# psipred/DMPfold2

Hardware: AMD Instinct MI355X
Metric: structures/s at L=300, N_seq=2000, 10 iters+100 min (higher is better)
Workload: dtype f32 with full-width operands on the bf16 matrix cores (option precision = 2): convolution operands split exactly into 3 bf16 pieces (24 significand bits), the 6 piece products above 2^-24 accumulated in f32 by v_mfma_f32_32x32x16_bf16; vertical GRU the same way (3 bf16 pieces per operand, 6 products

## Files before the change

dmpfold2_amd/csrc/api.hip:

```cpp
#include "cluster.h"
#include <atomic>
#include "conv_bf16.h"
#include "conv_f16.h"
#include <cstdarg>
#include <cstdio>
#include <cstring>
#include <cmath>

namespace dmp {

static thread_local char g_err[512] = "";

void set_error(const char* fmt, ...) {
  va_list ap;
  va_start(ap, fmt);
  vsnprintf(g_err, sizeof(g_err), fmt, ap);
  va_end(ap);
}

int hip_fail(hipError_t e, const char* what, const char* file, int line) {
  set_error("HIP error %d (%s) at %s:%d: %s", (int)e, hipGetErrorString(e), file, line, what);
  return DMP_ERR_HIP;
}

// ... 251 lines not shown
    }
    for (int q = 0; q < 128; ++q) {
      float a = 0.f;
      for (int r = 0; r < 8; ++r) a += w2[q * 8 + r] * hid[r];
      gate[q] = 1.0f / (1.0f + std::exp(-a));
    }
    if ((rc = upload(pool, bytes, &B.cse, gate))) return rc;
    {
      std::vector<float> fc(w1);
      fc.insert(fc.end(), w2.begin(), w2.end());
      if ((rc = upload(pool, bytes, &B.cse_fc, fc))) return rc;
    }
    if ((rc = upload(pool, bytes, &B.sse_w, H[p + ".scSE.sSE.conv.weight"]))) return rc;
    B.sse_b = H[p + ".scSE.sSE.conv.bias"][0];
  }
  if ((rc = upload(pool, bytes, &W.head_w, H["resnet.17.weight"]))) return rc;
  W.head_b[0] = H["resnet.17.bias"][0];
  W.head_b[1] = H["resnet.17.bias"][1];
  return DMP_OK;
}

static int check_ready(dmp_ctx* c, int L, int N) {
  if (!c) { set_error("null context"); return DMP_ERR_ARG; }
  if (L > c->max_L || N > c->max_N) {
    set_error("alignment %d x %d exceeds the context capacity %d x %d", N, L, c->max_N, c->max_L);
    return DMP_ERR_CAPACITY;
  }
  return DMP_OK;
}
static int need_weights(dmp_ctx* c) {
  if (!c->W.ready) { set_error("weights not finalized"); return DMP_ERR_WEIGHTS; }
  return DMP_OK;
}

static int trunk_open(dmp_ctx* c, const float* z0, const float* dmap, int L, hipStream_t s) {
  int rc;
  c->trunk_cur = c->xa;
  c->trunk_oth = c->xb;
  c->xsplit_current = false;
  c->ab_current = false;
  if ((rc = stem_update_padded(c, z0, dmap, L, c->trunk_cur, s, true))) return rc;
  c->xsplit_current = c->conv_mode != 1;
  return DMP_OK;
}

static int trunk_block(dmp_ctx* c, int k, int L, hipStream_t s) {
  int rc;
  {
    static const int depth = getenv("DMP_LANE_DEPTH") ? std::max(1, atoi(getenv("DMP_LANE_DEPTH"))) : 2;
    if (c->lane && c->lane->count >= depth)
      DMP_HIP(hipStreamWaitEvent(s, (hipEvent_t)c->lane->ev[(c->lane->count - depth) % dmp_lane::RING], 0));
  }
  if (c->prof_on && c->prof_n + 2 <= (int)c->prof_ev.size()) {
    DMP_HIP(hipEventRecord((hipEvent_t)c->prof_ev[c->prof_n], s));
  }
  if ((rc = conv5x5_maxout_padded(c, k, c->trunk_cur, L, c->u, c->stats, s, false))) return rc;
  if (c->lane) {
    dmp_lane* ln = c->lane;
    void* e = ln->ev[ln->next];
    ln->next = (ln->next + 1) % dmp_lane::RING;
    DMP_HIP(hipEventRecord((hipEvent_t)e, s));
    ln->last = e;
    ln->count++;
  }
  if (c->prof_on && c->prof_n + 2 <= (int)c->prof_ev.size()) {
    DMP_HIP(hipEventRecord((hipEvent_t)c->prof_ev[c->prof_n + 1], s));
    c->prof_n += 2;
  }
  if ((rc = conv5x5_reduce_stats(c, L, c->stats, s, k))) return rc;
  if ((rc = norm_scse_residual_padded(c, k, c->u, c->stats, c->trunk_cur, L, c->trunk_oth, s, k == NBLOCK))) return rc;
  std::swap(c->trunk_cur, c->trunk_oth);
  return DMP_OK;
}

static int trunk_close(dmp_ctx* c, int L, float* d_conf, float* d_M, hipStream_t s) {
  c->xsplit_current = false;
  return head_gram_padded(c, c->trunk_cur, L, d_conf, d_M, s);
}

static int trunk_pass(dmp_ctx* c, const float* z0, const float* dmap, int L, float* d_conf,
                      float* d_M, hipStream_t s) {
  struct Reset { dmp_ctx* c; ~Reset() { c->xsplit_current = false; } } reset{c};
  int rc;
  if ((rc = trunk_open(c, z0, dmap, L, s))) return rc;
  for (int k = 1; k <= NBLOCK; ++k)
    if ((rc = trunk_block(c, k, L, s))) return rc;
  return trunk_close(c, L, d_conf, d_M, s);
}

static int coords_from_mds(dmp_ctx* c, const float* mat1d, const float* mds, int L, float* d_ca,
                           hipStream_t s) {
  int rc;
  if ((rc = build_embed(mat1d, mds, L, c->emb, s))) return rc;
  if ((rc = gru_bidir(c, 1, c->emb, L, c->seq_a, s))) return rc;
  return coord_fc(c, c->seq_a, L, d_ca, s);
}

__global__ void fault_latch_kernel(int* __restrict__ words, float* __restrict__ coords,
                                   float* __restrict__ conf, int L, ConfLayout lay, int* __restrict__ report) {
  const int f = words[0];
  if (!f) return;
  const int64_t i = (int64_t)blockIdx.x * blockDim.x + threadIdx.x;
  const float nan = __builtin_nanf("");
  if (i < 15 * L) coords[i] = nan;
  if (conf_is_out(lay, i)) conf[i] = nan;
  if (i == 0) {
    atomicOr(&words[1], f);
    if (report) *report = f;
  }
}

static int scratch_reserve(dmp_ctx* c, Scratch& w, int64_t need, int64_t head, const char* what) {
  if (w.p && w.bytes >= need) return DMP_OK;
  int prev = 0;
  DMP_HIP(hipGetDevice(&prev));
  DMP_HIP(hipSetDevice(c->device));
  void* p = nullptr;
  hipError_t e = hipMalloc(&p, (size_t)need);
  if (e == hipSuccess) e = hipMemset(p, 0, (size_t)head);
  if (e == hipSuccess && w.p) e = hipFree(w.p);
  (void)hipSetDevice(prev);
  if (e != hipSuccess) {
    if (p) (void)hipFree(p);
    return hip_fail(e, what, __FILE__, __LINE__);
  }
  c->bytes += need - w.bytes;
  w = {(unsigned char*)p, need};
  return DMP_OK;
}
static int scratch_reserve(dmp_ctx* c, Scratch& w, ScratchNeed n, const char* what) { return scratch_reserve(c, w, n.bytes, n.head, what); }

static int search_reserve(dmp_ctx* c) {
  if (c->opt.search <= 0) return DMP_OK;
  const int mm = c->opt.search_mm > 0 ? c->opt.search_mm : c->max_L;
  int64_t need = 0;
  for (int L = 8; L <= c->max_L; ++L)
    need = std::max<int64_t>(need, (int64_t)search_chunk_entries(L, mm, 0) * search_slot(L, mm).total);
  return scratch_reserve(c, c->search_ws, SEARCH_HEAD_BYTES + need, SEARCH_HEAD_BYTES, "search scratch");
}
static int search_domains_reserve(dmp_ctx* c) {
  return c->opt.search_domains ? scratch_reserve(c, c->domsearch_ws, search_domains_need(c->max_L), "domain-search scratch") : DMP_OK;
}
static int passes_reserve(dmp_ctx* c) {
  return c->opt.passes ? scratch_reserve(c, c->pass_ws, score_passes_need(c->max_L), "pass-score scratch") : DMP_OK;
}
static int with_entity_reserve(dmp_ctx* c, Scratch& w, ScratchNeed n, const char* what) {
  const bool had = c->entity_ws.p != nullptr;
  int rc = scratch_reserve(c, c->entity_ws, entity_need(c->max_L), "native-entity scratch");
  if (!rc && (rc = scratch_reserve(c, w, n, what)) && !had) {
    (void)hipFree(c->entity_ws.p);
    c->bytes -= c->entity_ws.bytes;
    c->entity_ws = {};
  }
  return rc;
}
static int ss_reserve(dmp_ctx* c) {
  return c->opt.ss ? with_entity_reserve(c, c->ss_ws, assign_ss_need(c->max_L), "secondary-structure scratch") : DMP_OK;
}
static int exposure_reserve(dmp_ctx* c) {
  return c->opt.exposure ? with_entity_reserve(c, c->exposure_ws, exposure_need(c->max_L), "exposure scratch") : DMP_OK;
}
static int domains_reserve(dmp_ctx* c) {
  return c->opt.domains ? with_entity_reserve(c, c->domains_ws, domains_need(c->max_L), "domain scratch") : DMP_OK;
}

enum OptAccess { OPT_RW, OPT_READ_ONLY , OPT_GET_ONLY  };
// ... 973 lines not shown

int dmp_predict_end(dmp_ctx* ctx, float* d_coords, float* d_conf, void* stream) {
  DMP_ARG(ctx && d_coords && d_conf, "null argument");
  dmp_ctx* c = ctx;
  int rc = predict_end_refine(ctx, stream);
  if (rc) return rc;
  hipStream_t s = STREAM;
  const int L = c->last_L;
  rc = ca_to_backbone(c->best_ca, c->best_conf, L, d_coords, d_conf, s);
  if (rc) return rc;
  const int pass_R = c->run.passes ? std::min(c->run_depth + 1, c->max_passes) : 0;
  const ConfLayout lay = conf_layout(L, c->run, pass_R);
  if (c->run.emit && (rc = emit_distmap(c, c->best_ca, L, c->passes_done, d_conf + lay.map.off, d_conf + lay.info.off, s))) return rc;
  if (c->run.score && (rc = score_native(c, d_coords, L, d_conf + lay.score.off, s))) return rc;
  if (c->run.smap && (rc = score_map(c, L, d_conf + lay.score.off, d_conf + lay.smap.off, s))) return rc;
  if (pass_R && (rc = score_passes(c, L, pass_R, std::min(c->passes_done, c->max_passes), d_conf + lay.pass.off, s))) return rc;
  const float* d_native = c->run.score ? d_conf + lay.score.off : nullptr;
  const bool backbone = c->run.ss || c->run.exposure;
  if (d_native && (backbone || c->run.domains) && (rc = entity_prepare(c, d_native, L, backbone, s))) return rc;
  if (c->run.ss && (rc = assign_ss(c, d_coords, L, d_native, d_conf + lay.ss.off, s))) return rc;
  if (c->run.exposure && (rc = exposure(c, d_coords, L, d_native, d_conf + lay.exposure.off, s))) return rc;
  if (c->run.domains && (rc = domains(c, d_coords, L, d_native, d_conf + lay.domains.off, s))) return rc;
  if (c->run.align && (rc = align_structure(c, d_coords, L, d_conf + lay.align.off, s))) return rc;
  if (c->run.search > 0 && (rc = search_structures(c, d_coords, L, d_conf, lay, s))) return rc;
  if (c->run.search_domains && (rc = search_domains(c, d_coords, L, d_conf, lay, s))) return rc;
  hipLaunchKernelGGL(fault_latch_kernel, dim3((unsigned)cdiv64(std::max<int64_t>(15 * L, lay.total), 256)), dim3(256), 0, s,
                     c->seq_abort, d_coords, d_conf, L, lay, c->end_fault_out);
  DMP_LAUNCH_CHECK();
  return DMP_OK;
}

static std::shared_ptr<dmp_lane> lane_create() {
  std::shared_ptr<dmp_lane> l(new dmp_lane(), [](dmp_lane* p) {
    for (void* e : p->ev) (void)hipEventDestroy((hipEvent_t)e);
    delete p;
  });
  for (int i = 0; i < dmp_lane::RING; ++i) {
    hipEvent_t e;
    if (hipEventCreateWithFlags(&e, hipEventDisableTiming) != hipSuccess) return nullptr;
    l->ev.push_back((void*)e);
  }
  return l;
}

int dmp_ctx_share_lane(dmp_ctx* ctx, dmp_ctx* other) {
  DMP_ARG(ctx != nullptr, "null context");
  if (!other) { ctx->lane_hold.reset(); ctx->lane = nullptr; return DMP_OK; }
  DMP_ARG(other != ctx && other->device == ctx->device, "a lane is shared by different contexts of one GPU");
  if (!other->lane_hold) {
    other->lane_hold = lane_create();
    if (!other->lane_hold) { set_error("hipEventCreate failed for the lane"); return DMP_ERR_HIP; }
    other->lane = other->lane_hold.get();
  }
  ctx->lane_hold = other->lane_hold;
  ctx->lane = ctx->lane_hold.get();
  return DMP_OK;
}

int64_t dmp_debug_fetch(dmp_ctx* ctx, const char* name, float* d_dst, int64_t capacity, void* stream) {
  DMP_ARG(ctx && name && d_dst, "null argument");
  const int64_t L = ctx->last_L, N = ctx->last_N;
  const int64_t P = std::min(ctx->passes_done, ctx->max_passes);
  const float* src = nullptr;
  int64_t n = 0;
  const std::string k(name);
  if (k == "w") { src = ctx->w; n = N; }
  else if (k == "contacts") { src = ctx->contacts; n = L * L; }
  else if (k == "mat1d") { src = ctx->mat1d; n = WIDTH * L; }
  else if (k == "conf_means") { src = ctx->conf_means; n = P; }
  else if (k == "ca_pass") { src = ctx->ca_pass; n = P * L * 3; }
  else if (k == "pass_delta") { src = ctx->pass_delta; n = ctx->run.tol_mA > 0 ? P : 0; }
  else if (k == "best_dm") { src = ctx->best_dm; n = ctx->run.emit || ctx->run.restrain > 0 ? L * L : 0; }
  else if (k == "best_pass") { src = ctx->best_pass; n = 1; }
  else if (k == "best_ca") { src = ctx->best_ca_snapshot; n = L * 3; }
  else if (k == "best_ca_refined") { src = ctx->best_ca; n = L * 3; }
  else if (k == "inv_cov") { src = ctx->cov; n = (int64_t)NS * L * NS * L; }
  else if (k == "mds") { src = ctx->mds; n = L * 8; }
  else if (k == "gram") { src = ctx->gram; n = L * L; }
  else if (k == "vgru_h0" || k == "vgru_h1") {
    const int layer = k == "vgru_h1";
    src = ctx->hT[layer][ctx->vg_maxN & 1];
    n = (int64_t)WIDTH * ctx->vg_ntiles * 32;
  }
  else if (k == "exposure_points") return exposure_points_fetch(d_dst, capacity, STREAM);
  else if (k == "exposure_native_backbone") {
    const bool on = ctx->exposure_ws.p && ctx->run.exposure && ctx->run.score;
    src = on ? exposure_native_backbone(ctx) : nullptr;
    n = on ? 15 * L : 0;
  }
  else { set_error("unknown debug tensor %s", name); return DMP_ERR_ARG; }
  if (n > capacity) { set_error("capacity %lld too small for %s (%lld)", (long long)capacity, name, (long long)n); return DMP_ERR_ARG; }
  if (n > 0) DMP_HIP(hipMemcpyAsync(d_dst, src, sizeof(float) * n, hipMemcpyDeviceToDevice, STREAM));
  return n;
}

int dmp_profile_enable(dmp_ctx* ctx, int on, int max_launches) {
  DMP_ARG(ctx != nullptr, "null context");
  ctx->prof_on = on != 0;
  ctx->prof_n = 0;
  while ((int)ctx->prof_ev.size() < 2 * max_launches) {
    hipEvent_t e;
    DMP_HIP(hipEventCreate(&e));
    ctx->prof_ev.push_back((void*)e);
  }
  return DMP_OK;
}


int dmp_profile_conv_intervals(dmp_ctx* ctx, dmp_ctx* ref, float* h_start_ms, float* h_end_ms, int capacity,
                               int* h_launches) {
  DMP_ARG(ctx && ref && h_start_ms && h_end_ms && h_launches, "null argument");
  DMP_ARG(ref->prof_n >= 2, "the reference context has no recorded launch");
  const int n = ctx->prof_n / 2 < capacity ? ctx->prof_n / 2 : capacity;
  hipEvent_t e0 = (hipEvent_t)ref->prof_ev[0];
  for (int i = 0; i < n; ++i) {
    DMP_HIP(hipEventElapsedTime(&h_start_ms[i], e0, (hipEvent_t)ctx->prof_ev[2 * i]));
    DMP_HIP(hipEventElapsedTime(&h_end_ms[i], e0, (hipEvent_t)ctx->prof_ev[2 * i + 1]));
  }
  *h_launches = n;
  return DMP_OK;
}


}
```

dmpfold2_amd/csrc/common.h:

```cpp
#pragma once
#include <hip/hip_runtime.h>
#include <stdint.h>
#include <string>
#include <vector>
#include <map>
#include <algorithm>
#include <memory>
#include "../../include/dmpfold_hip.h"

struct TailOpts { int tol_mA = 0, emit = 0, score = 0, align = 0, search = 0, search_mm = 0, search_chunk = 0, search_refine = 0, smap = 0, passes = 0, passes_chunk = 0, ss = 0, restrain = 0, restrain_cut = 15000, exposure = 0, exposure_chunk = 0,
                  domains = 0, dom_tau = 250, dom_min_size = 40, dom_min_segment = 10, search_domains = 0; };

namespace dmp {

constexpr int WIDTH = 512;
constexpr int HID2 = 256;
constexpr float VGRU_STATE_SCALE = 1024.f;
constexpr int VGRU_CHUNK = 128;
constexpr int VGRU_CHUNK_SMALL = 16;
constexpr int CW = 128;
constexpr int NBLOCK = 16;
constexpr int STEM_OUT = 384;
constexpr int STEM_IN = 955;
constexpr int NS = 21;
// ... 228 lines not shown
  int cluster_local = 1;
  int tridiag_single = 0;
  int tridiag_cluster = 1;
  unsigned long long* tri_gx = nullptr;
  int refine_single = 0;
  int gj_diag_groups = 4;
  int gj_diag_blocked = 0;
  float* vout = nullptr;
  float* seq_g = nullptr;
  float* seq_a = nullptr;
  float* seq_b = nullptr;
  float* emb = nullptr;
  float* mat1d = nullptr;
  unsigned long long* seq_hx = nullptr;
  int* seq_abort = nullptr;
  unsigned long long* refine_gx = nullptr;
  int refine_xcd = 0;
  int seq_xcd0 = 0;
  float* z0 = nullptr;
  float* planes = nullptr;
  int planes_L = 0;
  bool planes_live = false;
  float* dmap = nullptr;
  float* u = nullptr;
  float* xa = nullptr;
  float* xb = nullptr;
  float* xdense = nullptr;
  uint16_t* xsplit = nullptr;
  int conv_mode = 2;
  int act_scaling = 1;
  bool xsplit_current = false;
  bool ab_current = false;
  double* part = nullptr;
  int part_count = 0;
  int conv_tile_bands = 0;
  double* stats = nullptr;
  float* ab = nullptr;
  float* bwd_ws = nullptr;
  int64_t bwd_ws_floats = 0;
  int bwd_w_block = 0;
  float* head0 = nullptr;
  float* head1 = nullptr;
  bool head_current = false;
  float* conf = nullptr;
  float* gram = nullptr;
  double* eig_a = nullptr;
  double* eig_ws = nullptr;
  float* mds = nullptr;
  float* ca = nullptr;
  float* best_ca = nullptr;
  float* best_conf = nullptr;
  float* best_mean = nullptr;
  float* conf_means = nullptr;
  float* ca_pass = nullptr;
  float* best_ca_snapshot = nullptr;
  int passes_done = 0;
  TailOpts opt;
  TailOpts run;
  int gate_pass = 0;
  float* delta_keep = nullptr;
  float* pass_delta = nullptr;
  double* delta_partial = nullptr;
  unsigned* delta_counter = nullptr;
  int* delta_host = nullptr;
  float* best_pass = nullptr;
  float* best_dm = nullptr;
  double* rms_partial = nullptr;
  unsigned* rms_counter = nullptr;
  dmp::Scratch score_ws;
  dmp::Scratch map_ws;
  dmp::Scratch align_ws;
  dmp::Scratch search_ws;
  dmp::Scratch pass_ws;
  dmp::Scratch entity_ws;
  dmp::Scratch ss_ws;
  dmp::Scratch exposure_ws;
  dmp::Scratch domains_ws;
  dmp::Scratch domsearch_ws;
  int search_last_L = 0, search_last_mm = 0, search_last_C = 0;
  int* end_fault_out = nullptr;
  bool end_refined = false;
  int unit_next = 0;
  float *trunk_cur = nullptr, *trunk_oth = nullptr;
  void* unit_ev[2] = {nullptr, nullptr};
  void* side_stream = nullptr;
  void* side_ev[2] = {nullptr, nullptr};
  bool fe_side = false;
  long unit_seq = 0;
  int fe_next = 0, fe_total = 0;
  int fe_inv = 0, fe_vgru = 0;
  const uint8_t* run_msa = nullptr;
  const float* run_template = nullptr;
  int last_L = 0, last_N = 0;
  int max_passes = 0;
  bool prof_on = false;
  int prof_n = 0;
  std::vector<void*> prof_ev;
};

namespace dmp {
struct GemmArgs {
  const float* A; int64_t sam, sak;
  const float* B; int64_t sbk, sbn;
  float* C; int64_t ldc;
  int M, N, K;
  float alpha, beta;
  const float* bias_n;
  bool lower_tiles;
};
int gemm_f32(const GemmArgs& g, hipStream_t s);

int msa_weights(dmp_ctx* c, const uint8_t* d_msa, int N, int L, float* d_w, hipStream_t s);
int cov_build(dmp_ctx* c, const uint8_t* d_msa, const float* d_w, int N, int L, float* d_cov,
              hipStream_t s, bool lower_only = false);
int trunk_kernel_attrs(dmp_ctx* c);
int spd_inverse(dmp_ctx* c, float* d_A, int D, hipStream_t s, hipStream_t la = nullptr);
int spd_inverse_steps(dmp_ctx* c, float* d_A, int D, int blk_lo, int blk_hi, hipStream_t s, hipStream_t la = nullptr);
int dca_contacts(dmp_ctx* c, const float* d_inv, int L, float* d_contacts, hipStream_t s);
int dca_features(const float* d_inv, const float* d_contacts, int L, float* d_out, hipStream_t s);
int gru_vertical(dmp_ctx* c, const uint8_t* d_msa, int N, int L, float* d_out, hipStream_t s);
int gru_vertical_steps(dmp_ctx* c, const uint8_t* d_msa, int N, int L, int t_lo, int t_hi, float* d_out,
                       hipStream_t s);
int vgru_kernel_attrs(dmp_ctx* c);
size_t vgru_x3_stream_bytes();
inline int vgru_runs_f32(const dmp_ctx* c) { return c->vgru_f32 >= 0 ? c->vgru_f32 : (c->conv_mode == 1 ? 1 : 0); }
class CoResident {
 public:
  CoResident(dmp_ctx* c, hipStream_t s, bool persistent);
  ~CoResident();
  int status() const { return rc_; }
  int done();
 private:
  dmp_ctx* c_; hipStream_t s_; bool persistent_, locked_; int rc_;
};
void coresident_forget(dmp_ctx* c);
int vgru_group_setup(dmp_ctx* lead, dmp_ctx* const* members, const uint8_t* const* msas, const int* Ns,
                     const int* Ls, int n, hipStream_t s);
int vgru_group_steps(dmp_ctx* lead, int t_lo, int t_hi, hipStream_t s);
int vgru_group_output(dmp_ctx* lead, int member_index, int N, int L, float* d_out, hipStream_t s, dmp_ctx* member = nullptr);
int gru_bidir(dmp_ctx* c, int which, const float* d_in, int T, float* d_out, hipStream_t s);
int stem_static(dmp_ctx* c, const float* d_mat1d, const float* d_inv, const float* d_contacts,
                int L, float* d_z0, hipStream_t s);
int stem_update_padded(dmp_ctx* c, const float* d_z0, const float* d_dmap, int L, float* d_xpad,
                       hipStream_t s, bool split = false);
int conv5x5_maxout_padded(dmp_ctx* c, int block, const float* d_xpad, int L, float* d_u,
                          double* d_stats, hipStream_t s, bool reduce);
int conv5x5_reduce_stats(dmp_ctx* c, int L, double* d_stats, hipStream_t s, int block = 0);
int conv5x5_maxout_winners(dmp_ctx* c, int block, const float* d_xpad, int L, float* d_u, uint8_t* d_idx, hipStream_t s);
int norm_scse_residual_padded(dmp_ctx* c, int block, const float* d_u, const double* d_stats,
                              const float* d_xpad_in, int L, float* d_xpad_out, hipStream_t s, bool head = false);
int conv5x5_maxout_fwd_winners(dmp_ctx* c, int block, const float* d_x, int L, float* d_u, uint8_t* d_idx, hipStream_t s);
int conv5x5_maxout_bwd(dmp_ctx* c, int block, const float* d_x, const float* d_du, const uint8_t* d_idx, int L, float* d_dx,
                       float* d_dw, float* d_db, hipStream_t s);
int norm_scse_residual_bwd(dmp_ctx* c, int block, const float* d_u, const float* d_dout, int L, float* d_du,
                           float* d_dparams, hipStream_t s);
int head_conv_bwd(dmp_ctx* c, const float* d_x, const float* d_g, int L, float* d_dx, float* d_dparams, hipStream_t s);
int stem_maxout_fwd_winners(dmp_ctx* c, const float* d_z0, const float* d_dmap, int L, float* d_u, uint8_t* d_idx, hipStream_t s);
int stem_bwd(dmp_ctx* c, const float* d_u, const uint8_t* d_idx, const float* d_dy, const float* d_mat1d, const float* d_dmap,
             int L, float* d_dw, float* d_dparams, float* d_dmat1d, hipStream_t s);
int head_gram_padded(dmp_ctx* c, const float* d_xpad, int L, float* d_conf, float* d_M,
                     hipStream_t s);
int act_pad(const float* d_dense, int L, float* d_xpad, hipStream_t s);
int act_unpad(const float* d_xpad, int L, float* d_dense, hipStream_t s);
int act_clear(float* d_xpad, int L, hipStream_t s);
int act_split(dmp_ctx* c, const float* d_xpad, int L, int block, hipStream_t s);
__device__ __forceinline__ float gate_exp(float x) {
// ... 139 lines not shown
```

dmpfold2_amd/csrc/conv_bf16.h:

```cpp
#pragma once
#include "conv_split.h"

namespace dmp {

typedef __bf16 cq_bf16x8 __attribute__((ext_vector_type(8)));

#ifndef CQ_PITCH_N
#define CQ_PITCH_N 20
#endif
template <int NQ> using CqShape = CsShape<NQ, 3, CQ_PITCH_N>;
template <int NQ> constexpr int convq_lds_bytes() { return 2 * CqShape<NQ>::IN_BYTES; }
constexpr int CONVQ_LDS_BYTES = convq_lds_bytes<8>();

__host__ __device__ inline uint16_t cq_bf16_rne(float f) {
  uint32_t u = __builtin_bit_cast(uint32_t, f);
  u += 0x7FFFu + ((u >> 16) & 1u);
  return (uint16_t)(u >> 16);
}
__host__ __device__ inline float cq_bf16_f32(uint16_t h) {
  return __builtin_bit_cast(float, (uint32_t)h << 16);
}
__host__ __device__ inline void split3_bf16(float x, uint16_t p[3]) {
  p[0] = cq_bf16_rne(x);
  const float r1 = x - cq_bf16_f32(p[0]);
  p[1] = cq_bf16_rne(r1);
  const float r2 = r1 - cq_bf16_f32(p[1]);
  p[2] = cq_bf16_rne(r2);
}

inline std::vector<uint16_t> pack_conv_weights_bf16(const float* w) {
  return conv_split_pack_weights<3>(w, [](float x, uint16_t* p) { split3_bf16(x, p); });
}

#if defined(__HIPCC__) && defined(CONV_BF16_KERNELS)
__device__ __forceinline__ cs_f32x16 cq_mfma(uint4 a, uint4 b, cs_f32x16 c) {
  return __builtin_amdgcn_mfma_f32_32x32x16_bf16(__builtin_bit_cast(cq_bf16x8, a),
                                                 __builtin_bit_cast(cq_bf16x8, b), c, 0, 0, 0);
}

template <int NQ, int NT, int PAR, class MID>
__device__ __forceinline__ void cq_column_pass(const uint4 (&a)[NT][3], const uint4* il, cs_f32x16 (&acc)[NQ], MID&& mid) {
  constexpr int PIECE = CqShape<NQ>::PIECE, RP = CqShape<NQ>::RP, PITCH = CqShape<NQ>::PITCH;
  uint4 bn0 = il[PAR * PITCH], bn1 = il[PAR * PITCH + PIECE], bn2 = il[PAR * PITCH + 2 * PIECE];
#pragma unroll
  for (int r = PAR; r < RP; r += 2) {
    const uint4 b0 = bn0, b1 = bn1, b2 = bn2;
    if (r + 2 < RP) {
      bn0 = il[(r + 2) * PITCH];
      bn1 = il[(r + 2) * PITCH + PIECE];
      bn2 = il[(r + 2) * PITCH + 2 * PIECE];
    }
#define CQ_TAPS(AP, BV)                                                           \
    _Pragma("unroll") for (int t = 0; t < NT; ++t) {                              \
      const int q = (r - PAR - 2 * t) / 2;                                        \
      if (r - PAR - 2 * t >= 0 && q < NQ) acc[q] = cq_mfma(a[t][AP], BV, acc[q]); \
    }
    CQ_TAPS(0, b2)
    CQ_TAPS(1, b1)
    CQ_TAPS(2, b0)
    CQ_TAPS(0, b1)
    CQ_TAPS(1, b0)
    CQ_TAPS(0, b0)
#undef CQ_TAPS
    if (r == PAR + 2 * (NT - 1)) mid();
  }
}

template <int NT>
__device__ __forceinline__ void cq_load_weights(const uint4* __restrict__ src, uint4 (&a)[NT][3]) {
#pragma unroll
  for (int t = 0; t < NT; ++t)
#pragma unroll
    for (int p = 0; p < 3; ++p) a[t][p] = src[t * CqShape<8>::WSLOT + p * 64];
}

#ifdef CQ_CLOCK_STAMPS
constexpr int CQ_STAMP_BLOCKS = 2048;
__device__ unsigned long long cq_clock_stamps[CQ_STAMP_BLOCKS][2];
#endif

template <int NQ>
__global__ __launch_bounds__(256, 2) void conv5x5_bf16x6_kernel(const uint16_t* __restrict__ xs,
                                                                const uint16_t* __restrict__ wq,
                                                                const float* __restrict__ bias, int L, int P,
                                                                int tiles, int nwork, float* __restrict__ u,
                                                                double* __restrict__ part) {
  using SH = CqShape<NQ>;
  const int id = blockIdx.x, tid = threadIdx.x;
  const CsBlock blk = cs_block<NQ>(id, tiles);
  if (blk.none) return;
  CsLane ln = cs_lane(tid);
  if (NQ == 4 && blk.ty0 >= L) {
    cs_zero_sums(blk, ln, part);
    return;
  }
  cs_lane_pixel(ln.li, ln.prow, ln.px);
  const int wave = ln.wave;
  const int64_t PP = (int64_t)P * P;

  const uint4* in_l = reinterpret_cast<const uint4*>(cs_smem);
  const unsigned lds_base = (unsigned)(size_t)(__attribute__((address_space(3))) unsigned char*)cs_smem;

  const uint4* xs4 = reinterpret_cast<const uint4*>(xs);
  int in_src[SH::IN_PAD / 256 + 1];
#pragma unroll
  for (int e = 0; e <= SH::IN_PAD / 256; ++e) in_src[e] = cs_halo_src<SH>(e * 256 + tid, P, blk);
  auto tile_dma = [&](int g) {
    cs_tile_dma<SH>(xs4 + (int64_t)g * 2 * PP, lds_base + (g & 1) * SH::IN_BYTES, wave, [&](int e) { return in_src[e]; });
  };
  const uint4* wcol = reinterpret_cast<const uint4*>(wq) + (int64_t)blk.split * 8 * 5 * 4 * SH::WCOL +
                      (int64_t)wave * SH::WCOL + ln.lane;
  const int b_base = (ln.kk * SH::HALO + ln.prow) * SH::PITCH + ln.px;

  cs_f32x16 acc[NQ];
#pragma unroll
  for (int q = 0; q < NQ; ++q)
#pragma unroll
    for (int r = 0; r < 16; ++r) acc[q][r] = 0.f;

  uint4 ae[3][3], ao[2][3];
  tile_dma(0);
  cq_load_weights<3>(wcol, ae);
  __builtin_amdgcn_sched_barrier(0);
#ifdef CQ_CLOCK_STAMPS
  const unsigned long long st_clk = __builtin_amdgcn_s_memtime(), st_real = __builtin_amdgcn_s_memrealtime();
#endif

  for (int g = 0; g < 8; ++g) {
    cs_wait_vm<0>();
    __syncthreads();
    const uint4* in_g = in_l + (g & 1) * SH::IN_PAD + b_base;
#pragma unroll 1
    for (int dx = 0; dx < 5; ++dx) {
      const uint4* il = in_g + dx;
      {
        __builtin_amdgcn_sched_barrier(0);
        cq_load_weights<2>(wcol + 3 * SH::WSLOT, ao);
        __builtin_amdgcn_sched_barrier(0);
        cq_column_pass<NQ, 3, 0>(ae, il, acc, [&] {
          if (dx == 0 && g < 7) {
            __builtin_amdgcn_sched_barrier(0);
            tile_dma(g + 1);
            __builtin_amdgcn_sched_barrier(0);
          }
        });
      }
      {
        const uint4* wnext = wcol + (g * 5 + dx < 39 ? 4 * SH::WCOL : 0);
        __builtin_amdgcn_sched_barrier(0);
        cq_load_weights<3>(wnext, ae);
        __builtin_amdgcn_sched_barrier(0);
        cq_column_pass<NQ, 2, 1>(ao, il, acc, [] {});
        wcol = wnext;
      }
    }
  }
#ifdef CQ_CLOCK_STAMPS
  if (tid == 0 && id < CQ_STAMP_BLOCKS) {
    cq_clock_stamps[id][0] = __builtin_amdgcn_s_memtime() - st_clk;
    cq_clock_stamps[id][1] = __builtin_amdgcn_s_memrealtime() - st_real;
  }
#endif

  cs_epilogue<false>(acc, bias, blk, ln, L, u, part);
}
#endif

}
```

dmpfold2_amd/csrc/trunk.hip:

```cpp
#include "common.h"
#include <type_traits>
#define CONV_BF16_KERNELS
#include "conv_bf16.h"
#define CONV_F16_KERNELS
#include "conv_f16.h"

#pragma clang fp contract(off)

namespace dmp {

typedef float f32x16 __attribute__((ext_vector_type(16)));

__device__ __forceinline__ float sigmoid_f(float x) { return 1.0f / (1.0f + expf(-x)); }

template <int MODE>
__device__ __forceinline__ void store_pieces(const float (&o)[8], uint16_t* __restrict__ xs, int64_t slot,
                                             int64_t piece_stride, int* __restrict__ fault, float xscale) {
  constexpr int NP = (MODE == 0) ? 2 : 3;
  uint16_t pc[NP][8];
  bool bad = false;
#pragma unroll
  for (int e = 0; e < 8; ++e) {
    if constexpr (MODE == 0) {
      uint16_t p2[2];
// ... 531 lines not shown
  float o[8];
#pragma unroll
  for (int e = 0; e < 8; ++e) o[e] = xpad[(int64_t)(cgp * 8 + e) * PP + (int64_t)y * P + x];
  store_pieces<MODE>(o, xs, (int64_t)cgp * PP + (int64_t)y * P + x, 16 * PP, fault, xscale);
}

int act_split(dmp_ctx* c, const float* d_xpad, int L, int block, hipStream_t s) {
  const int P = act_pitch(L);
  dim3 grid(cdiv(P, 256), P, 16);
  if (c->conv_mode == 2)
    hipLaunchKernelGGL(act_split_kernel<2>, grid, dim3(256), 0, s, d_xpad, P, c->xsplit, c->seq_abort, 1.0f);
  else
    hipLaunchKernelGGL(act_split_kernel<0>, grid, dim3(256), 0, s, d_xpad, P, c->xsplit, c->seq_abort,
                       c->act_scaling ? c->W.blk[block - 1].x_scale : 1.0f);
  DMP_LAUNCH_CHECK();
  return DMP_OK;
}

int trunk_kernel_attrs(dmp_ctx* c) {
  static bool done[64] = {};
  if (c->device >= 0 && c->device < 64 && done[c->device]) return DMP_OK;
  auto lds = [](const void* k, int bytes) { return hipFuncSetAttribute(k, hipFuncAttributeMaxDynamicSharedMemorySize, bytes); };
  DMP_HIP(lds((const void*)conv5x5_bf16x6_kernel<8>, convq_lds_bytes<8>()));
  DMP_HIP(lds((const void*)conv5x5_bf16x6_kernel<4>, convq_lds_bytes<4>()));
  DMP_HIP(lds((const void*)conv5x5_f16x3_kernel<8>, convh_lds_bytes<8>()));
  DMP_HIP(lds((const void*)conv5x5_f16x3_kernel<4>, convh_lds_bytes<4>()));
  if (c->device >= 0 && c->device < 64) done[c->device] = true;
  return DMP_OK;
}

int conv5x5_maxout_padded(dmp_ctx* c, int block, const float* d_xpad, int L, float* d_u,
                          double* d_stats, hipStream_t s, bool reduce) {
  const BlockW& B = c->W.blk[block - 1];
  const int tiles = act_tiles(L), P = act_pitch(L);
  const int nwork = tiles * tiles * CONV_SPLIT;
  const int grid = round_up(nwork, 8);
  if (c->conv_mode != 1) {
    if (!c->xsplit_current) {
      int rc = act_split(c, d_xpad, L, block, s);
      if (rc) return rc;
    }
    const int bands = c->conv_tile_bands > 0 ? c->conv_tile_bands : conv_split_rows(tiles);
    const float scale = c->act_scaling ? B.wh_inv_scale / B.x_scale : B.wh_inv_scale;
    if (c->conv_mode == 2) {
      if (bands == 2)
        hipLaunchKernelGGL(conv5x5_bf16x6_kernel<4>, dim3(conv_split_grid(tiles, 2)), dim3(256), convq_lds_bytes<4>(), s,
                           c->xsplit, B.wq, B.bias, L, P, tiles, nwork, d_u, c->part);
      else
        hipLaunchKernelGGL(conv5x5_bf16x6_kernel<8>, dim3(conv_split_grid(tiles, 1)), dim3(256), convq_lds_bytes<8>(), s,
                           c->xsplit, B.wq, B.bias, L, P, tiles, nwork, d_u, c->part);
    } else {
      if (bands == 2)
        hipLaunchKernelGGL(conv5x5_f16x3_kernel<4>, dim3(conv_split_grid(tiles, 2)), dim3(256), convh_lds_bytes<4>(), s,
                           c->xsplit, B.wh, B.bias, scale, L, P, tiles, nwork, d_u, c->part);
      else
        hipLaunchKernelGGL(conv5x5_f16x3_kernel<8>, dim3(conv_split_grid(tiles, 1)), dim3(256), convh_lds_bytes<8>(), s,
                           c->xsplit, B.wh, B.bias, scale, L, P, tiles, nwork, d_u, c->part);
    }
    DMP_LAUNCH_CHECK();
    c->part_count = 2 * tiles * tiles;
    return reduce ? conv5x5_reduce_stats(c, L, d_stats, s) : DMP_OK;
  }
  hipLaunchKernelGGL(conv5x5_maxout_kernel<false>, dim3(grid), dim3(256), 0, s, d_xpad, B.wpack, B.bias, L,
                     P, tiles, nwork, d_u, c->part, (uint8_t*)nullptr);
  DMP_LAUNCH_CHECK();
  c->part_count = tiles * tiles;
  return reduce ? conv5x5_reduce_stats(c, L, d_stats, s) : DMP_OK;
}

int conv5x5_maxout_winners(dmp_ctx* c, int block, const float* d_xpad, int L, float* d_u, uint8_t* d_idx, hipStream_t s) {
  const BlockW& B = c->W.blk[block - 1];
  const int tiles = act_tiles(L), P = act_pitch(L);
  const int nwork = tiles * tiles * CONV_SPLIT;
  hipLaunchKernelGGL(conv5x5_maxout_kernel<true>, dim3(round_up(nwork, 8)), dim3(256), 0, s, d_xpad, B.wpack, B.bias, L,
                     P, tiles, nwork, d_u, c->part, d_idx);
  DMP_LAUNCH_CHECK();
  c->part_count = tiles * tiles;
  return DMP_OK;
}

#ifndef NORM_PRIO
#define NORM_PRIO 0
#endif
template <int SPLIT, int HEAD>
__global__ __launch_bounds__(256) void norm_scse_residual_kernel(
    const float* __restrict__ u, const float* __restrict__ ab, const float* __restrict__ cse,
    const float* __restrict__ sse_w, float sse_b, const float* __restrict__ xin, int L, int P,
    float* __restrict__ xout, uint16_t* __restrict__ xs, int* __restrict__ fault, float xscale,
    const float* __restrict__ hw, float hb0, float hb1, float* __restrict__ head0, float* __restrict__ head1) {
  __shared__ float sh_a[CW], sh_b[CW], sh_g[CW], sh_w[CW], sh_h[HEAD ? 2 * CW : 1];
#if NORM_PRIO
  __builtin_amdgcn_s_setprio(NORM_PRIO);
#endif
  if (threadIdx.x < CW) {
    sh_a[threadIdx.x] = ab[threadIdx.x * 2];
    sh_b[threadIdx.x] = ab[threadIdx.x * 2 + 1];
    sh_g[threadIdx.x] = cse[threadIdx.x];
    sh_w[threadIdx.x] = sse_w[threadIdx.x];
  }
  if constexpr (HEAD) sh_h[threadIdx.x] = hw[threadIdx.x];
  __syncthreads();
  const int lane = threadIdx.x & 63, wave = threadIdx.x >> 6;
  const int q = lane >> 4;
  const int y = blockIdx.y;
  const int x = blockIdx.x * 64 + wave * 16 + (lane & 15);
  const bool live = x < L;
  const int xc = live ? x : L - 1;
  const int64_t LL = (int64_t)L * L, PP = (int64_t)P * P;
  const int64_t p = (int64_t)y * L + xc, pp = (int64_t)(y + 2) * P + xc + 2;
  constexpr int QC = CW / 4;
  float yv[QC];
  float dot = 0.f;
#pragma unroll
  for (int i = 0; i < QC; ++i) {
    const int c = q * QC + i;
    yv[i] = u[c * LL + p] * sh_a[c] + sh_b[c];
    dot = fmaf(sh_w[c], yv[i], dot);
  }
  dot += __shfl_xor(dot, 16, 64);
  dot += __shfl_xor(dot, 32, 64);
  const float sg = sigmoid_f(dot + sse_b);
  float h0 = 0.f, h1 = 0.f;
#pragma unroll
  for (int g8 = 0; g8 < QC / 8; ++g8) {
    const int cgp = q * (QC / 8) + g8;
    float o[8];
#pragma unroll
    for (int e = 0; e < 8; ++e) {
      const int c = cgp * 8 + e;
      const float t = yv[g8 * 8 + e] * sh_g[c] + yv[g8 * 8 + e] * sg;
      o[e] = t + xin[c * PP + pp];
      if (live) xout[c * PP + pp] = o[e];
      if constexpr (HEAD) {
        h0 = fmaf(sh_h[c], o[e], h0);
        h1 = fmaf(sh_h[CW + c], o[e], h1);
      }
    }
    if (live) {
      if constexpr (SPLIT == 0) store_pieces<0>(o, xs, (int64_t)cgp * PP + pp, 16 * PP, fault, xscale);
      if constexpr (SPLIT == 2) store_pieces<2>(o, xs, (int64_t)cgp * PP + pp, 16 * PP, fault, 1.0f);
    }
  }
  if constexpr (HEAD) {
    h0 += __shfl_xor(h0, 16, 64);
    h0 += __shfl_xor(h0, 32, 64);
    h1 += __shfl_xor(h1, 16, 64);
    h1 += __shfl_xor(h1, 32, 64);
    if (live && q == 0) {
      head0[(int64_t)y * L + x] = h0 + hb0;
      head1[(int64_t)y * L + x] = h1 + hb1;
    }
  }
}

int norm_scse_residual_padded(dmp_ctx* c, int block, const float* d_u, const double* d_stats,
                              const float* d_xpad_in, int L, float* d_xpad_out, hipStream_t s, bool head) {
  const BlockW& B = c->W.blk[block - 1];
  const Weights& W = c->W;
  const int P = act_pitch(L);
  if (!c->ab_current) {
    hipLaunchKernelGGL(norm_coeff_kernel, dim3(1), dim3(CW), 0, s, d_stats, (double)L * (double)L,
                       B.gamma, B.beta, c->ab);
    DMP_LAUNCH_CHECK();
  }
  c->ab_current = false;
  const int split = (c->conv_mode != 1 && c->xsplit_current && block < NBLOCK) ? c->conv_mode : -1;
  const float xscale = (c->act_scaling && block < NBLOCK) ? c->W.blk[block].x_scale : 1.0f;
  dim3 grid(cdiv(L, 64), L);
#define NORM_LAUNCH(S, H)                                                                              \
  hipLaunchKernelGGL((norm_scse_residual_kernel<S, H>), grid, dim3(256), 0, s, d_u, c->ab, B.cse, B.sse_w, \
                     B.sse_b, d_xpad_in, L, P, d_xpad_out, c->xsplit, c->seq_abort, xscale, W.head_w,   \
                     W.head_b[0], W.head_b[1], c->head0, c->head1)
  if (head) NORM_LAUNCH(-1, 1);
  else if (split == 0) NORM_LAUNCH(0, 0);
  else if (split == 2) NORM_LAUNCH(2, 0);
  else NORM_LAUNCH(-1, 0);
#undef NORM_LAUNCH
  DMP_LAUNCH_CHECK();
  c->head_current = head;
  return DMP_OK;
}

__global__ __launch_bounds__(256) void head_planes_kernel(const float* __restrict__ xpad,
                                                          const float* __restrict__ hw, float b0, float b1,
                                                          int L, int P, float* __restrict__ head0,
                                                          float* __restrict__ head1) {
  __shared__ float sw[2 * CW];
  sw[threadIdx.x] = hw[threadIdx.x];
  __syncthreads();
  const int i = blockIdx.y;
  const int j = blockIdx.x * 256 + threadIdx.x;
  if (j >= L) return;
  const int64_t PP = (int64_t)P * P;
  const float* px = xpad + (int64_t)(i + 2) * P + j + 2;
  float p0[4], p1[4];
#pragma unroll
  for (int q = 0; q < 4; ++q) {
    p0[q] = 0.f; p1[q] = 0.f;
#pragma unroll 8
    for (int k = 0; k < CW / 4; ++k) {
      const int c = q * (CW / 4) + k;
      const float v = px[c * PP];
      p0[q] = fmaf(sw[c], v, p0[q]);
      p1[q] = fmaf(sw[CW + c], v, p1[q]);
    }
  }
  head0[(int64_t)i * L + j] = ((p0[0] + p0[1]) + (p0[2] + p0[3])) + b0;
  head1[(int64_t)i * L + j] = ((p1[0] + p1[1]) + (p1[2] + p1[3])) + b1;
}

__global__ __launch_bounds__(256) void head_conf_kernel(const float* __restrict__ head1, int L,
                                                        float* __restrict__ conf) {
  __shared__ double red[256];
  const int i = blockIdx.x;
  double rsum = 0.0;
  for (int j = threadIdx.x; j < L; j += 256) rsum += (double)head1[(int64_t)i * L + j];
  const double total = block_tree_sum_f64<256>(rsum, red);
  if (threadIdx.x == 0) conf[i] = (float)(total / (double)L);
}

__global__ __launch_bounds__(256) void gram_kernel(const float* __restrict__ h0, int L,
                                                   float* __restrict__ M) {
  const int i = blockIdx.y;
  const int j = blockIdx.x * 256 + threadIdx.x;
  if (j >= L) return;
  auto dm = [&](int a, int b) {
    return distmap_entry(h0[(int64_t)a * L + b], h0[(int64_t)b * L + a]);
  };
  const float d0j = dm(0, j), di0 = dm(i, 0), dij = dm(i, j);
  const float t = d0j * d0j + di0 * di0;
  M[(int64_t)i * L + j] = 0.5f * (t - dij * dij);
}

int head_gram_padded(dmp_ctx* c, const float* d_xpad, int L, float* d_conf, float* d_M,
                     hipStream_t s) {
  const Weights& W = c->W;
  const int P = act_pitch(L);
  if (!c->head_current) {
    hipLaunchKernelGGL(head_planes_kernel, dim3(cdiv(L, 256), L), dim3(256), 0, s, d_xpad, W.head_w, W.head_b[0],
                       W.head_b[1], L, P, c->head0, c->head1);
    DMP_LAUNCH_CHECK();
  }
  c->head_current = false;
  hipLaunchKernelGGL(head_conf_kernel, dim3(L), dim3(256), 0, s, c->head1, L, d_conf);
  DMP_LAUNCH_CHECK();
  hipLaunchKernelGGL(gram_kernel, dim3(cdiv(L, 256), L), dim3(256), 0, s, c->head0, L, d_M);
  DMP_LAUNCH_CHECK();
  return DMP_OK;
}

}

#ifdef CQ_CLOCK_STAMPS
extern "C" int dmp_debug_conv_clock(unsigned long long* host, int blocks) {
  if (!host || blocks < 1 || blocks > dmp::CQ_STAMP_BLOCKS) return -1;
  if (hipDeviceSynchronize() != hipSuccess) return -1;
  return hipMemcpyFromSymbol(host, HIP_SYMBOL(dmp::cq_clock_stamps), sizeof(unsigned long long) * 2 * blocks) == hipSuccess ? 0 : -1;
}
#endif
// ... 1 lines not shown
```

Measured before the change: 4.480.

## Skip dead-row MFMAs in edge conv tiles and widen norm kernel pixels per wave

```diff
diff --git a/dmpfold2_amd/csrc/api.hip b/dmpfold2_amd/csrc/api.hip
--- a/dmpfold2_amd/csrc/api.hip
+++ b/dmpfold2_amd/csrc/api.hip
@@ -357,6 +357,7 @@
                       float* d_M, hipStream_t s) {
   struct Reset { dmp_ctx* c; ~Reset() { c->xsplit_current = false; } } reset{c};
   int rc;
+  c->trunk_L = L;
   if ((rc = trunk_open(c, z0, dmap, L, s))) return rc;
   for (int k = 1; k <= NBLOCK; ++k)
     if ((rc = trunk_block(c, k, L, s))) return rc;
@@ -1496,6 +1497,18 @@
     src = ctx->hT[layer][ctx->vg_maxN & 1];
     n = (int64_t)WIDTH * ctx->vg_ntiles * 32;
   }
+  else if (k.rfind("trunk_", 0) == 0) {
+    const int64_t TL = ctx->trunk_L, TP = TL ? act_pitch((int)TL) : 0;
+    if (k == "trunk_x") { src = ctx->trunk_cur; n = CW * TP * TP; }
+    else if (k == "trunk_x15") { src = ctx->trunk_oth; n = CW * TP * TP; }
+    else if (k == "trunk_pieces") {
+      src = reinterpret_cast<const float*>(ctx->xsplit);
+      n = ctx->conv_mode == 1 ? 0 : (ctx->conv_mode == 0 ? 2 : 3) * 16 * TP * TP * 4;
+    }
+    else if (k == "trunk_head0") { src = ctx->head0; n = TL * TL; }
+    else if (k == "trunk_head1") { src = ctx->head1; n = TL * TL; }
+    else { set_error("unknown debug tensor %s", name); return DMP_ERR_ARG; }
+  }
   else if (k == "exposure_points") return exposure_points_fetch(d_dst, capacity, STREAM);
   else if (k == "exposure_native_backbone") {
     const bool on = ctx->exposure_ws.p && ctx->run.exposure && ctx->run.score;
diff --git a/dmpfold2_amd/csrc/common.h b/dmpfold2_amd/csrc/common.h
--- a/dmpfold2_amd/csrc/common.h
+++ b/dmpfold2_amd/csrc/common.h
@@ -334,6 +334,7 @@
   bool end_refined = false;
   int unit_next = 0;
   float *trunk_cur = nullptr, *trunk_oth = nullptr;
+  int trunk_L = 0;
   void* unit_ev[2] = {nullptr, nullptr};
   void* side_stream = nullptr;
   void* side_ev[2] = {nullptr, nullptr};
diff --git a/dmpfold2_amd/csrc/conv_bf16.h b/dmpfold2_amd/csrc/conv_bf16.h
--- a/dmpfold2_amd/csrc/conv_bf16.h
+++ b/dmpfold2_amd/csrc/conv_bf16.h
@@ -1,5 +1,6 @@
 #pragma once
 #include "conv_split.h"
+#include <type_traits>
 
 namespace dmp {
 
@@ -7,6 +8,9 @@
 
 #ifndef CQ_PITCH_N
 #define CQ_PITCH_N 20
+#endif
+#ifndef CQ_LIVE_ROWS
+#define CQ_LIVE_ROWS 1
 #endif
 template <int NQ> using CqShape = CsShape<NQ, 3, CQ_PITCH_N>;
 template <int NQ> constexpr int convq_lds_bytes() { return 2 * CqShape<NQ>::IN_BYTES; }
@@ -38,9 +42,11 @@
                                                  __builtin_bit_cast(cq_bf16x8, b), c, 0, 0, 0);
 }
 
-template <int NQ, int NT, int PAR, class MID>
+template <int NQ, int NL, int NT, int PAR, class MID>
 __device__ __forceinline__ void cq_column_pass(const uint4 (&a)[NT][3], const uint4* il, cs_f32x16 (&acc)[NQ], MID&& mid) {
-  constexpr int PIECE = CqShape<NQ>::PIECE, RP = CqShape<NQ>::RP, PITCH = CqShape<NQ>::PITCH;
+  constexpr int PIECE = CqShape<NQ>::PIECE, PITCH = CqShape<NQ>::PITCH;
+  constexpr int RP = CqShape<NQ>::RP < PAR + 2 * (NL + NT - 1) ? CqShape<NQ>::RP : PAR + 2 * (NL + NT - 1);
+  static_assert(NL >= 1 && NL <= NQ, "live accumulators");
   uint4 bn0 = il[PAR * PITCH], bn1 = il[PAR * PITCH + PIECE], bn2 = il[PAR * PITCH + 2 * PIECE];
 #pragma unroll
   for (int r = PAR; r < RP; r += 2) {
@@ -53,7 +59,7 @@
 #define CQ_TAPS(AP, BV)                                                           \
     _Pragma("unroll") for (int t = 0; t < NT; ++t) {                              \
       const int q = (r - PAR - 2 * t) / 2;                                        \
-      if (r - PAR - 2 * t >= 0 && q < NQ) acc[q] = cq_mfma(a[t][AP], BV, acc[q]); \
+      if (r - PAR - 2 * t >= 0 && q < NL) acc[q] = cq_mfma(a[t][AP], BV, acc[q]); \
     }
     CQ_TAPS(0, b2)
     CQ_TAPS(1, b1)
@@ -119,41 +125,53 @@
     for (int r = 0; r < 16; ++r) acc[q][r] = 0.f;
 
   uint4 ae[3][3], ao[2][3];
-  tile_dma(0);
-  cq_load_weights<3>(wcol, ae);
-  __builtin_amdgcn_sched_barrier(0);
 #ifdef CQ_CLOCK_STAMPS
   const unsigned long long st_clk = __builtin_amdgcn_s_memtime(), st_real = __builtin_amdgcn_s_memrealtime();
 #endif
 
-  for (int g = 0; g < 8; ++g) {
-    cs_wait_vm<0>();
-    __syncthreads();
-    const uint4* in_g = in_l + (g & 1) * SH::IN_PAD + b_base;
+  auto stages = [&](auto nl) __attribute__((always_inline)) {
+    constexpr int NL = decltype(nl)::value;
+    tile_dma(0);
+    cq_load_weights<3>(wcol, ae);
+    __builtin_amdgcn_sched_barrier(0);
+    for (int g = 0; g < 8; ++g) {
+      cs_wait_vm<0>();
+      __syncthreads();
+      const uint4* in_g = in_l + (g & 1) * SH::IN_PAD + b_base;
 #pragma unroll 1
-    for (int dx = 0; dx < 5; ++dx) {
-      const uint4* il = in_g + dx;
-      {
-        __builtin_amdgcn_sched_barrier(0);
-        cq_load_weights<2>(wcol + 3 * SH::WSLOT, ao);
-        __builtin_amdgcn_sched_barrier(0);
-        cq_column_pass<NQ, 3, 0>(ae, il, acc, [&] {
-          if (dx == 0 && g < 7) {
-            __builtin_amdgcn_sched_barrier(0);
-            tile_dma(g + 1);
-            __builtin_amdgcn_sched_barrier(0);
-          }
-        });
-      }
-      {
-        const uint4* wnext = wcol + (g * 5 + dx < 39 ? 4 * SH::WCOL : 0);
-        __builtin_amdgcn_sched_barrier(0);
-        cq_load_weights<3>(wnext, ae);
-        __builtin_amdgcn_sched_barrier(0);
-        cq_column_pass<NQ, 2, 1>(ao, il, acc, [] {});
-        wcol = wnext;
+      for (int dx = 0; dx < 5; ++dx) {
+        const uint4* il = in_g + dx;
+        {
+          __builtin_amdgcn_sched_barrier(0);
+          cq_load_weights<2>(wcol + 3 * SH::WSLOT, ao);
+          __builtin_amdgcn_sched_barrier(0);
+          cq_column_pass<NQ, NL, 3, 0>(ae, il, acc, [&] {
+            if (dx == 0 && g < 7) {
+              __builtin_amdgcn_sched_barrier(0);
+              tile_dma(g + 1);
+              __builtin_amdgcn_sched_barrier(0);
+            }
+          });
+        }
+        {
+          const uint4* wnext = wcol + (g * 5 + dx < 39 ? 4 * SH::WCOL : 0);
+          __builtin_amdgcn_sched_barrier(0);
+          cq_load_weights<3>(wnext, ae);
+          __builtin_amdgcn_sched_barrier(0);
+          cq_column_pass<NQ, NL, 2, 1>(ao, il, acc, [] {});
+          wcol = wnext;
+        }
       }
     }
+  };
+  if constexpr (NQ == 8 && CQ_LIVE_ROWS) {
+    const int live = L - blk.ty0;
+    if (live > 12) stages(std::integral_constant<int, 8>());
+    else if (live > 8) stages(std::integral_constant<int, 6>());
+    else if (live > 4) stages(std::integral_constant<int, 4>());
+    else stages(std::integral_constant<int, 2>());
+  } else {
+    stages(std::integral_constant<int, NQ>());
   }
 #ifdef CQ_CLOCK_STAMPS
   if (tid == 0 && id < CQ_STAMP_BLOCKS) {
diff --git a/dmpfold2_amd/csrc/trunk.hip b/dmpfold2_amd/csrc/trunk.hip
--- a/dmpfold2_amd/csrc/trunk.hip
+++ b/dmpfold2_amd/csrc/trunk.hip
@@ -637,12 +637,19 @@
 #ifndef NORM_PRIO
 #define NORM_PRIO 0
 #endif
-template <int SPLIT, int HEAD>
+#ifndef NORM_LANES_BF16
+#define NORM_LANES_BF16 2
+#endif
+template <int SPLIT, int HEAD, int LPP>
 __global__ __launch_bounds__(256) void norm_scse_residual_kernel(
     const float* __restrict__ u, const float* __restrict__ ab, const float* __restrict__ cse,
     const float* __restrict__ sse_w, float sse_b, const float* __restrict__ xin, int L, int P,
     float* __restrict__ xout, uint16_t* __restrict__ xs, int* __restrict__ fault, float xscale,
     const float* __restrict__ hw, float hb0, float hb1, float* __restrict__ head0, float* __restrict__ head1) {
+  static_assert(LPP == 2 || LPP == 4, "lanes per pixel");
+  constexpr int PIX = 64 / LPP;
+  constexpr int NQL = 4 / LPP;
+  constexpr int QC = CW / 4;
   __shared__ float sh_a[CW], sh_b[CW], sh_g[CW], sh_w[CW], sh_h[HEAD ? 2 * CW : 1];
 #if NORM_PRIO
   __builtin_amdgcn_s_setprio(NORM_PRIO);
@@ -656,29 +663,38 @@
   if constexpr (HEAD) sh_h[threadIdx.x] = hw[threadIdx.x];
   __syncthreads();
   const int lane = threadIdx.x & 63, wave = threadIdx.x >> 6;
-  const int q = lane >> 4;
+  if ((blockIdx.x * 4 + wave) * PIX >= L) return;
+  const int q = lane / PIX;
   const int y = blockIdx.y;
-  const int x = blockIdx.x * 64 + wave * 16 + (lane & 15);
+  const int x = (blockIdx.x * 4 + wave) * PIX + (lane & (PIX - 1));
   const bool live = x < L;
   const int xc = live ? x : L - 1;
   const int64_t LL = (int64_t)L * L, PP = (int64_t)P * P;
   const int64_t p = (int64_t)y * L + xc, pp = (int64_t)(y + 2) * P + xc + 2;
-  constexpr int QC = CW / 4;
-  float yv[QC];
-  float dot = 0.f;
-#pragma unroll
-  for (int i = 0; i < QC; ++i) {
-    const int c = q * QC + i;
-    yv[i] = u[c * LL + p] * sh_a[c] + sh_b[c];
-    dot = fmaf(sh_w[c], yv[i], dot);
-  }
-  dot += __shfl_xor(dot, 16, 64);
+  float yv[NQL * QC];
+  float dq[NQL];
+#pragma unroll
+  for (int k = 0; k < NQL; ++k) {
+    dq[k] = 0.f;
+#pragma unroll
+    for (int i = 0; i < QC; ++i) {
+      const int c = (q * NQL + k) * QC + i;
+      yv[k * QC + i] = u[c * LL + p] * sh_a[c] + sh_b[c];
+      dq[k] = fmaf(sh_w[c], yv[k * QC + i], dq[k]);
+    }
+  }
+  float dot = dq[0];
+  if constexpr (LPP == 2) dot += dq[NQL - 1];
+  if constexpr (LPP == 4) dot += __shfl_xor(dot, 16, 64);
   dot += __shfl_xor(dot, 32, 64);
   const float sg = sigmoid_f(dot + sse_b);
-  float h0 = 0.f, h1 = 0.f;
-#pragma unroll
-  for (int g8 = 0; g8 < QC / 8; ++g8) {
-    const int cgp = q * (QC / 8) + g8;
+  float hq0[NQL], hq1[NQL];
+#pragma unroll
+  for (int k = 0; k < NQL; ++k) hq0[k] = hq1[k] = 0.f;
+#pragma unroll
+  for (int g8 = 0; g8 < NQL * QC / 8; ++g8) {
+    const int cgp = q * (NQL * QC / 8) + g8;
+    const int k = g8 / (QC / 8);
     float o[8];
 #pragma unroll
     for (int e = 0; e < 8; ++e) {
@@ -687,8 +703,8 @@
       o[e] = t + xin[c * PP + pp];
       if (live) xout[c * PP + pp] = o[e];
       if constexpr (HEAD) {
-        h0 = fmaf(sh_h[c], o[e], h0);
-        h1 = fmaf(sh_h[CW + c], o[e], h1);
+        hq0[k] = fmaf(sh_h[c], o[e], hq0[k]);
+        hq1[k] = fmaf(sh_h[CW + c], o[e], hq1[k]);
       }
     }
     if (live) {
@@ -697,9 +713,16 @@
     }
   }
   if constexpr (HEAD) {
-    h0 += __shfl_xor(h0, 16, 64);
+    float h0 = hq0[0], h1 = hq1[0];
+    if constexpr (LPP == 2) {
+      h0 += hq0[NQL - 1];
+      h1 += hq1[NQL - 1];
+    }
+    if constexpr (LPP == 4) {
+      h0 += __shfl_xor(h0, 16, 64);
+      h1 += __shfl_xor(h1, 16, 64);
+    }
     h0 += __shfl_xor(h0, 32, 64);
-    h1 += __shfl_xor(h1, 16, 64);
     h1 += __shfl_xor(h1, 32, 64);
     if (live && q == 0) {
       head0[(int64_t)y * L + x] = h0 + hb0;
@@ -721,15 +744,19 @@
   c->ab_current = false;
   const int split = (c->conv_mode != 1 && c->xsplit_current && block < NBLOCK) ? c->conv_mode : -1;
   const float xscale = (c->act_scaling && block < NBLOCK) ? c->W.blk[block].x_scale : 1.0f;
-  dim3 grid(cdiv(L, 64), L);
-#define NORM_LAUNCH(S, H)                                                                              \
-  hipLaunchKernelGGL((norm_scse_residual_kernel<S, H>), grid, dim3(256), 0, s, d_u, c->ab, B.cse, B.sse_w, \
-                     B.sse_b, d_xpad_in, L, P, d_xpad_out, c->xsplit, c->seq_abort, xscale, W.head_w,   \
+#define NORM_LAUNCH(S, H, LPP)                                                                                      \
+  hipLaunchKernelGGL((norm_scse_residual_kernel<S, H, LPP>), dim3(cdiv(L, 256 / LPP), L), dim3(256), 0, s, d_u, c->ab, \
+                     B.cse, B.sse_w, B.sse_b, d_xpad_in, L, P, d_xpad_out, c->xsplit, c->seq_abort, xscale, W.head_w, \
                      W.head_b[0], W.head_b[1], c->head0, c->head1)
-  if (head) NORM_LAUNCH(-1, 1);
-  else if (split == 0) NORM_LAUNCH(0, 0);
-  else if (split == 2) NORM_LAUNCH(2, 0);
-  else NORM_LAUNCH(-1, 0);
+  if (c->conv_mode == 2) {
+    if (head) NORM_LAUNCH(-1, 1, NORM_LANES_BF16);
+    else if (split == 2) NORM_LAUNCH(2, 0, NORM_LANES_BF16);
+    else NORM_LAUNCH(-1, 0, NORM_LANES_BF16);
+  } else {
+    if (head) NORM_LAUNCH(-1, 1, 4);
+    else if (split == 0) NORM_LAUNCH(0, 0, 4);
+    else NORM_LAUNCH(-1, 0, 4);
+  }
 #undef NORM_LAUNCH
   DMP_LAUNCH_CHECK();
   c->head_current = head;
```

New measurement: 4.498 (median of 6 runs). Within noise of the previous version (+0.4%).
